# fzi-forschungszentrum-informatik/muvo

Hardware: AMD Instinct MI355X
Metric: world-model training samples/sec (seq_len=10) (higher is better)
Workload: dtype f32 storage/accumulate; large contractions (convolutions, transformer Linear) as bf16x3 split products

## Files before the change

### muvo_amd/csrc/conv_bf3.h

```cpp
#pragma once
#include "conv_plan.h"

void bf3_finish_phase(ConvPhase& g);
int bf3_pack_phase(const ConvPhase& g, const float* w, float* wp, hipStream_t st);
long bf3_workspace_bytes(int N, int C, long S);
int bf3_split_input(const float* x, void* ws, int N, int C, long S, hipStream_t st, const float* yact = nullptr, int act = 0,
                    float slope = 0.f, float* dbias = nullptr, const float* dhead = nullptr, const float* head_w = nullptr, int CO = 0,
                    float* dhead_w = nullptr, float* dhead_b = nullptr);
int bf3_launch_fwd_phase(const ConvPhase& g, const void* ws, const float* wp, const float* bias, float* out, int act,
                         float slope, hipStream_t st, int ksplit = 1);
void bf3_set_fused_head(const float* w, const float* b, float* out, int co);
void bf3_set_products(int n);
int bf3_get_products();
int bf3_fwd_ksplit(const ConvPhase& g);
int bf3_wgrad_phase(const ConvPhase& g, const void* ws_x, int Cin_total, const void* ws_dz, int Cout_total, float* wg,
                    float* dw, hipStream_t st);
int bf3_split_rows(const float* x, void* ws, long rows, int C, hipStream_t st);
bool bf3_fwd_uses_pp(const ConvPhase& g);
bool bf3_wgrad_uses_pp(const ConvPhase& g);
struct PackItem {
  ConvPhase g;
  const float* w;
  float* dst;
  long blk0;
  int nblk, pad_;
};
int pack_table_launch(const PackItem* dev_items, int n, long n_blocks, hipStream_t st);
```

### muvo_amd/csrc/conv_bf3.hip

```cpp
#include "conv_bf3.h"
#include <type_traits>

typedef __bf16 bf16x8 __attribute__((ext_vector_type(8)));
typedef __bf16 bf16x2 __attribute__((ext_vector_type(2)));
typedef float f32x2 __attribute__((ext_vector_type(2)));

__device__ unsigned long long g_bf3_clock[3];
extern "C" int muvo_bf3_loop_clock(double* shader_mhz, double* us_per_k_step) {
  unsigned long long h[3] = {0, 0, 0};
  if (hipMemcpyFromSymbol(h, HIP_SYMBOL(g_bf3_clock), sizeof(h)) != hipSuccess) return MUVO_ERR_HIP;
  if (h[1] == 0 || h[2] == 0) { *shader_mhz = 0.0; *us_per_k_step = 0.0; return MUVO_OK; }
  *shader_mhz = (double)h[0] / ((double)h[1] / 100.0);
  *us_per_k_step = (double)h[1] / 100.0 / (double)h[2];
  return MUVO_OK;
}

#ifdef MUVO_BF3_STAMPS
__device__ unsigned long long g_bf3_stamps[8 * 16384];
#define BF3_STAMP(slot)                                                                      \
  if (MUVO_BF3_STAMPS != 3 && threadIdx.x == 0 && blockIdx.x < 16384) g_bf3_stamps[blockIdx.x * 8 + (slot)] = __builtin_amdgcn_s_memrealtime()
extern "C" int muvo_debug_bf3_stamps_reset() {
  void* p = nullptr;
  return hipGetSymbolAddress(&p, HIP_SYMBOL(g_bf3_stamps)) == hipSuccess && hipMemset(p, 0, sizeof(unsigned long long) * 8 * 16384) == hipSuccess ? 0 : 1;
}
// ... 1250 lines not shown
    hipLaunchKernelGGL(nchw_split_nhwc_v4_kernel, grid, dim3(256), lds, st, x, hi, lo, C, Cp, S, yact, act, slope, dbias ? rep : nullptr,
                       dhead, head_w, CO, hw_rep, nrep);
  } else {
    hipLaunchKernelGGL(nchw_split_nhwc_kernel, grid, dim3(256), 0, st, x, hi, lo, C, Cp, S, yact, act, slope, rep, nrep);
  }
  if (dbias) hipLaunchKernelGGL(bias_replica_reduce_kernel, dim3(cdiv(Cp, 64)), dim3(64), 0, st, rep, dbias, C, Cp, nrep);
  if (hw_rep) hipLaunchKernelGGL(head_replica_reduce_kernel, dim3(cdiv(4 * Cp + 4, 64)), dim3(64), 0, st, hw_rep, dhead_w, dhead_b, C, Cp, CO, nrep);
  MUVO_CHECK_LAUNCH("nchw_split_nhwc_kernel");
  return MUVO_OK;
}

__global__ void __launch_bounds__(256) rows_split_kernel(const float* __restrict__ in, uint4* __restrict__ out_hi,
                                                         uint4* __restrict__ out_lo, long n_u4) {
  for (long i = blockIdx.x * 256L + threadIdx.x; i < n_u4; i += (long)gridDim.x * 256) {
    const float4 a = reinterpret_cast<const float4*>(in)[2 * i], b = reinterpret_cast<const float4*>(in)[2 * i + 1];
    uint4 h, l;
    split2(a.x, a.y, h.x, l.x);
    split2(a.z, a.w, h.y, l.y);
    split2(b.x, b.y, h.z, l.z);
    split2(b.z, b.w, h.w, l.w);
    out_hi[i] = h;
    out_lo[i] = l;
  }
  if (blockIdx.x == 0 && threadIdx.x == 0) out_hi[2 * n_u4] = make_uint4(0u, 0u, 0u, 0u);
}

int bf3_split_rows(const float* x, void* ws, long rows, int C, hipStream_t st) {
  const long n_u4 = rows * C / 8;
  uint4* hi = (uint4*)ws;
  hipLaunchKernelGGL(rows_split_kernel, dim3(ew_grid(n_u4)), dim3(256), 0, st, x, hi, hi + n_u4, n_u4);
  MUVO_CHECK_LAUNCH("rows_split_kernel");
  return MUVO_OK;
}

struct Bf3Head { const float* w; const float* b; float* out; int co; };
static thread_local Bf3Head t_bf3_head = {nullptr, nullptr, nullptr, 0};

static int g_bf3_products = 3;
void bf3_set_products(int n) { g_bf3_products = n == 1 ? 1 : 3; }
int bf3_get_products() { return g_bf3_products; }

template <int BM, int BN, int WM, int WN, int BKC, int NST, bool ONE>
static int bf3_launch_t(const ConvPhase& g, const void* ws, const float* wp, const float* bias, float* out, int act,
                        float slope, hipStream_t st, int ksplit) {
  constexpr size_t lds0 = (size_t)NST * 2 * BKC * (BM + BN) * 16 + 512 + 4 * BM * WN;
  static_assert(lds0 <= 160 * 1024, "LDS budget");
  constexpr size_t HEAD_LDS = NST == 3 ? 4096 : 0;
  const Bf3Head hd = (NST == 3 && ksplit <= 1) ? t_bf3_head : Bf3Head{nullptr, nullptr, nullptr, 0};
  const size_t lds = lds0 + (hd.co > 0 ? HEAD_LDS : 0);
  static_assert(lds0 + HEAD_LDS <= 160 * 1024, "LDS budget with a fused head");
  static bool attr_set = false;
  static const uint4* zero16 = nullptr;
  if (!attr_set) {
    if (hipFuncSetAttribute((const void*)conv_bf3_kernel<BM, BN, WM, WN, BKC, NST, ONE>, hipFuncAttributeMaxDynamicSharedMemorySize,
                            (int)(lds0 + HEAD_LDS)) != hipSuccess ||
        hipGetSymbolAddress((void**)&zero16, HIP_SYMBOL(g_zero16)) != hipSuccess) {
      muvo_set_error("conv_bf3: kernel attribute / symbol setup failed");
      return MUVO_ERR_HIP;
    }
    attr_set = true;
  }
  const long plane_u4 = (long)g.N * g.ID * g.IH * g.IW * (g.Cp / 8);
  dim3 grid(cdiv(g.npix, BN) * cdiv(g.M, BM), ksplit, 1);
  hipLaunchKernelGGL((conv_bf3_kernel<BM, BN, WM, WN, BKC, NST, ONE>), grid, dim3(64 * WM * WN), lds, st, g, (const uint4*)ws, plane_u4,
                     (const uint4*)wp, bias, out, act, slope, zero16, ksplit, hd.w, hd.b, hd.out, hd.co);
  MUVO_CHECK_LAUNCH("conv_bf3_kernel");
  return MUVO_OK;
}
template <int BM, int BN, int WM, int WN, int BKC, int NST>
static int bf3_launch(const ConvPhase& g, const void* ws, const float* wp, const float* bias, float* out, int act,
                      float slope, hipStream_t st, int ksplit = 1) {
  return g_bf3_products == 1 ? bf3_launch_t<BM, BN, WM, WN, BKC, NST, true>(g, ws, wp, bias, out, act, slope, st, ksplit)
                             : bf3_launch_t<BM, BN, WM, WN, BKC, NST, false>(g, ws, wp, bias, out, act, slope, st, ksplit);
}

bool bf3_fwd_uses_pp(const ConvPhase& g) {
  if (g.M <= 64) return false;
  const long big = g.M > 128 ? (long)cdiv(g.npix, 128) * cdiv(g.M, 256) : (long)cdiv(g.npix, 256) * cdiv(g.M, 128);
  static const int min_blocks = getenv("MUVO_BF3_PP_MIN_BLOCKS") ? atoi(getenv("MUVO_BF3_PP_MIN_BLOCKS")) : 128;
  return big >= min_blocks;
}
bool bf3_wgrad_uses_pp(const ConvPhase& g) { return g.M > 128 || (g.M > 64 && g.C > 64); }

int bf3_fwd_ksplit(const ConvPhase& g) {
  if (g.npix <= 0 || bf3_fwd_uses_pp(g) || muvo_det()) return 1;
  static const int tgt = getenv("MUVO_BF3_KSPLIT_BLOCKS") ? atoi(getenv("MUVO_BF3_KSPLIT_BLOCKS")) : 512;
  static const int min_steps = getenv("MUVO_BF3_KSPLIT_MIN_STEPS") ? atoi(getenv("MUVO_BF3_KSPLIT_MIN_STEPS")) : 16;
  const long tiles = (long)cdiv(g.npix, 128) * cdiv(g.M, 64);
  const int nk = g.Kp / 32;
  if (tiles >= 192 || nk < 2 * min_steps) return 1;
  int ks = cdiv(tgt, tiles);
  if (ks > nk / min_steps) ks = nk / min_steps;
  return ks < 1 ? 1 : ks;
}

void bf3_set_fused_head(const float* w, const float* b, float* out, int co) { t_bf3_head = Bf3Head{w, b, out, co}; }

int bf3_launch_fwd_phase(const ConvPhase& g, const void* ws, const float* wp, const float* bias, float* out, int act,
                         float slope, hipStream_t st, int ksplit) {
  if (g.npix <= 0) return MUVO_OK;
  if (ksplit > 1) return bf3_launch<64, 128, 1, 4, 4, 2>(g, ws, wp, nullptr, out, MUVO_ACT_NONE, 0.f, st, ksplit);
  static const int variant = getenv("MUVO_BF3_VARIANT") ? atoi(getenv("MUVO_BF3_VARIANT")) : 0;
  if (variant == 2) {
    if (g.M > 128) return bf3_launch<256, 128, 4, 2, 4, 2>(g, ws, wp, bias, out, act, slope, st);
    if (g.M > 64) return bf3_launch<128, 256, 2, 4, 4, 2>(g, ws, wp, bias, out, act, slope, st);
  }
  if (bf3_fwd_uses_pp(g)) {
    if (g.M > 128) return bf3_launch<256, 128, 4, 2, 4, 3>(g, ws, wp, bias, out, act, slope, st);
    return bf3_launch<128, 256, 2, 4, 4, 3>(g, ws, wp, bias, out, act, slope, st);
  }
  return bf3_launch<64, 128, 1, 4, 4, 2>(g, ws, wp, bias, out, act, slope, st);
}

static int bf3_wgrad_ksplit(long tiles, int nsteps, int tgt, int minst, int slots) {
  if (muvo_det()) return 1;
  int ksplit = cdiv(tgt, tiles);
  if (ksplit > cdiv(nsteps, minst)) ksplit = cdiv(nsteps, minst);
  if (ksplit < 1) ksplit = 1;
  static const int quant = getenv("MUVO_BF3_WGRAD_QUANT") ? atoi(getenv("MUVO_BF3_WGRAD_QUANT")) : 1;
  if (quant && tiles * ksplit < 4L * slots) {
    const int kmax = nsteps / 12 > 1 ? nsteps / 12 : 1;
    double best = 1e30;
    for (int ks = 1; ks <= kmax && tiles * ks <= 8L * slots; ++ks) {
      const int sps = cdiv(nsteps, ks);
      if (cdiv(nsteps, sps) != ks) continue;
      const double cost = (double)cdiv(tiles * ks, slots) * (sps * 1.2 + 12.0);
      if (cost < best - 1e-9) { best = cost; ksplit = ks; }
    }
  }
  return ksplit;
}

static int bf3_wgrad_xcd_order() {
  static const int v = getenv("MUVO_BF3_WGRAD_XCD") ? atoi(getenv("MUVO_BF3_WGRAD_XCD")) : 1;
  return v;
}

template <int BM, int BN, int WM, int WN, bool ONE>
static int bf3_wgrad_pp_launch_t(const ConvPhase& g, const void* ws_x, int Cin_total, const void* ws_dz, int Cout_total,
                                 float* wg, hipStream_t st) {
  constexpr size_t lds = (size_t)3 * 2 * 32 * (BM / 8 + BN / 8) * 16;
  static bool attr_set = false;
  if (!attr_set) {
    if (hipFuncSetAttribute((const void*)conv_bf3_wgrad_pp_kernel<BM, BN, WM, WN, ONE>, hipFuncAttributeMaxDynamicSharedMemorySize,
                            (int)lds) != hipSuccess) {
      muvo_set_error("conv_bf3_wgrad_pp: kernel attribute setup failed");
      return MUVO_ERR_HIP;
    }
    attr_set = true;
  }
  ConvPhase p = g;
  const int xc8 = roundup(Cin_total, 8) / 8, dzc8 = roundup(Cout_total, 8) / 8;
  p.Cp = xc8 * 8;
  const long xplane = (long)g.N * g.ID * g.IH * g.IW * xc8, dzplane = (long)g.N * g.OD * g.OH * g.OW * dzc8;
  const int ctiles = cdiv(g.C, BN), mtiles = cdiv(g.M, BM);
  const int nsteps = cdiv(g.npix, 32);
  static const int tgt = getenv("MUVO_BF3_WGRAD_PP_BLOCKS") ? atoi(getenv("MUVO_BF3_WGRAD_PP_BLOCKS")) : 2048;
  static const int minst = getenv("MUVO_BF3_WGRAD_PP_MINSTEPS") ? atoi(getenv("MUVO_BF3_WGRAD_PP_MINSTEPS")) : 32;
  int ksplit = bf3_wgrad_ksplit((long)ctiles * g.T * mtiles, nsteps, tgt, minst, 256);
  const int sps = cdiv(nsteps, ksplit);
  ksplit = cdiv(nsteps, sps);
  dim3 grid(ctiles * g.T, mtiles, ksplit);
  hipLaunchKernelGGL((conv_bf3_wgrad_pp_kernel<BM, BN, WM, WN, ONE>), grid, dim3(64 * WM * WN), lds, st, p, (const uint4*)ws_x, xplane,
                     xc8, (const uint4*)ws_dz, dzplane, dzc8, wg, sps, bf3_wgrad_xcd_order());
  MUVO_CHECK_LAUNCH("conv_bf3_wgrad_pp_kernel");
  return MUVO_OK;
}
template <int BM, int BN, int WM, int WN>
static int bf3_wgrad_pp_launch(const ConvPhase& g, const void* ws_x, int Cin_total, const void* ws_dz, int Cout_total,
                               float* wg, hipStream_t st) {
  return g_bf3_products == 1 ? bf3_wgrad_pp_launch_t<BM, BN, WM, WN, true>(g, ws_x, Cin_total, ws_dz, Cout_total, wg, st)
                             : bf3_wgrad_pp_launch_t<BM, BN, WM, WN, false>(g, ws_x, Cin_total, ws_dz, Cout_total, wg, st);
}

template <int BM, int BN, int WM, int WN, int WK, bool ONE>
static int bf3_wgrad_launch_t(const ConvPhase& g, const void* ws_x, int Cin_total, const void* ws_dz, int Cout_total,
                              float* wg, hipStream_t st) {
  constexpr size_t lds = (size_t)3 * 2 * 32 * (BM / 8 + BN / 8) * 16;
  static bool attr_set = false;
  static const uint4* zero16 = nullptr;
  if (!attr_set) {
    if (hipFuncSetAttribute((const void*)conv_bf3_wgrad_kernel<BM, BN, WM, WN, WK, ONE>, hipFuncAttributeMaxDynamicSharedMemorySize,
                            (int)lds) != hipSuccess ||
        hipGetSymbolAddress((void**)&zero16, HIP_SYMBOL(g_zero16)) != hipSuccess) {
// ... 65 lines not shown
```

### muvo_amd/csrc/conv_gemm.hip

```cpp
#include "common.h"
#include "conv_vox.h"
#include "conv_pw.h"
#include "conv_plan.h"
#include "conv_bf3.h"

typedef __bf16 wg_bf16x8 __attribute__((ext_vector_type(8)));
__device__ __forceinline__ void wg_split8(const float (&v)[8], wg_bf16x8& hi, wg_bf16x8& lo) {
  typedef __bf16 b2 __attribute__((ext_vector_type(2)));
  typedef float f2 __attribute__((ext_vector_type(2)));
  unsigned h[4], l[4];
#pragma unroll
  for (int p = 0; p < 4; ++p) {
    const b2 hh = __builtin_convertvector((f2){v[2 * p], v[2 * p + 1]}, b2);
    h[p] = __builtin_bit_cast(unsigned, hh);
    const float h0 = __uint_as_float(h[p] << 16), h1 = __uint_as_float(h[p] & 0xffff0000u);
    const b2 ll = __builtin_convertvector((f2){v[2 * p] - h0, v[2 * p + 1] - h1}, b2);
    l[p] = __builtin_bit_cast(unsigned, ll);
  }
  typedef unsigned u4 __attribute__((ext_vector_type(4)));
  hi = __builtin_bit_cast(wg_bf16x8, (u4){h[0], h[1], h[2], h[3]});
  lo = __builtin_bit_cast(wg_bf16x8, (u4){l[0], l[1], l[2], l[3]});
}

template <int BM, int BN, int WM, int WN, int RUN>
// ... 566 lines not shown
        int k = 0;
        while (k < nu && uni[k] != phs[i].tap_d[t]) ++k;
        if (k == nu) { if (nu < MAX_TAPS) uni[nu++] = phs[i].tap_d[t]; else fits = false; }
      }
    static const int min_pct = getenv("MUVO_MERGE_UNION_MIN_PCT") ? atoi(getenv("MUVO_MERGE_UNION_MIN_PCT")) : 50;
    const bool merge = same_grid && (same_taps || (allow_union && fits && nu > 1 && 100 * real >= min_pct * count * nu));
    if (merge) {
      ConvPhase g = phs[0];
      g.nmerge = count;
      g.Msub = M;
      g.M = count * M;
      g.T = nu;
      for (int t = 0; t < nu; ++t) g.tap_d[t] = uni[t];
      for (int i = 0; i < count; ++i) {
        for (int a = 0; a < 3; ++a) g.mop[i][a] = phs[i].op[a];
        for (int t = 0; t < nu; ++t) {
          int k = 0;
          while (k < phs[i].T && phs[i].tap_d[k] != uni[t]) ++k;
          g.tap_wm[i][t] = k < phs[i].T ? phs[i].tap_w[k] : -1;
        }
      }
      for (int t = 0; t < nu; ++t) g.tap_w[t] = g.tap_wm[0][t] >= 0 ? g.tap_wm[0][t] : 0;
      finish_phase(g);
      phs[0] = g;
      count = 1;
    }
  }
  *nph = count;
  return MUVO_OK;
}

struct ConvPlan {
  ConvPhase fwd[8]; int nfwd;
  ConvPhase dgr[8]; int ndgr;
  long fwd_floats, dgr_floats;
};

static int build_plan(const muvo_conv_desc* d, ConvPlan* pl, int mode = -1, bool allow_merge = true) {
  int rc = check_desc(d);
  if (rc) return rc;
  t_plan_mode = mode < 0 ? conv_mode() : mode;
  t_allow_merge = allow_merge;
  const long taps = (long)d->ksz[0] * d->ksz[1] * d->ksz[2];
  if (!d->transposed) {
    pl->nfwd = 1;
    rc = build_conv_form(d, d->in_sz, d->out_sz, d->Cin, d->Cout, d->Cin * taps, taps, &pl->fwd[0]);
    if (rc) return rc;
    rc = build_transposed_form(d, d->out_sz, d->in_sz, d->Cout, d->Cin, taps, d->Cin * taps, pl->dgr, &pl->ndgr);
    if (rc) return rc;
  } else {
    rc = build_transposed_form(d, d->in_sz, d->out_sz, d->Cin, d->Cout, taps, d->Cout * taps, pl->fwd, &pl->nfwd);
    if (rc) return rc;
    pl->ndgr = 1;
    rc = build_conv_form(d, d->out_sz, d->in_sz, d->Cout, d->Cin, d->Cout * taps, taps, &pl->dgr[0]);
    if (rc) return rc;
  }
  long off = 0;
  for (int i = 0; i < pl->nfwd; ++i) { pl->fwd[i].wp_off = off; off += (long)pl->fwd[i].Kp * pl->fwd[i].Mp; }
  pl->fwd_floats = off;
  off = 0;
  for (int i = 0; i < pl->ndgr; ++i) { pl->dgr[i].wp_off = off; off += (long)pl->dgr[i].Kp * pl->dgr[i].Mp; }
  pl->dgr_floats = off;
  return MUVO_OK;
}

static double f32_bf3_min_gflop() {
  static const double v = getenv("MUVO_F32_BF3_MIN_GFLOP") ? atof(getenv("MUVO_F32_BF3_MIN_GFLOP")) : 2.0;
  return v;
}

template <int BM, int BN, int WM, int WN>
static void launch_fwd_run(const ConvPhase& g, const float* in, const float* wp, const float* bias, float* out,
                           int act, float slope, hipStream_t st, int ksplit) {
  dim3 grid(cdiv(g.npix, BN), cdiv(g.M, BM), ksplit);
  constexpr int KPT = 16 / (256 / BN);
  if (g.Cp == 4)
    hipLaunchKernelGGL((conv_fwd_kernel<BM, BN, WM, WN, 4>), grid, dim3(256), 0, st, g, in, wp, bias, out, act, slope, ksplit);
  else if (g.Cp == 8 || KPT == 8)
    hipLaunchKernelGGL((conv_fwd_kernel<BM, BN, WM, WN, 8>), grid, dim3(256), 0, st, g, in, wp, bias, out, act, slope, ksplit);
  else
    hipLaunchKernelGGL((conv_fwd_kernel<BM, BN, WM, WN, KPT>), grid, dim3(256), 0, st, g, in, wp, bias, out, act, slope, ksplit);
}

static int phase_ksplit(const ConvPhase& g) {
  if (g.npix <= 0 || muvo_det()) return 1;
  if (g.bf3) return bf3_fwd_ksplit(g);
  const int bm = g.M > 64 ? 128 : (g.M > 32 ? 64 : 32);
  const long blocks = (long)cdiv(g.npix, 128) * cdiv(g.M, bm);
  const int nk = g.Kp / 16;
  static const int min_steps = getenv("MUVO_KSPLIT_MIN_STEPS") ? atoi(getenv("MUVO_KSPLIT_MIN_STEPS")) : 8;
  if (blocks >= 192 || nk < 4 * min_steps) return 1;
  static const int ks_tgt = getenv("MUVO_KSPLIT_BLOCKS") ? atoi(getenv("MUVO_KSPLIT_BLOCKS")) : 384;
  int ks = cdiv(ks_tgt, blocks);
  if (ks > nk / min_steps) ks = nk / min_steps;
  return ks < 1 ? 1 : ks;
}

static int launch_fwd_phase(const ConvPhase& g, const float* in, const float* wp, const float* bias, float* out,
                            int act, float slope, hipStream_t st, const void* ws, int ksplit) {
  if (g.npix <= 0) return MUVO_OK;
  if (g.bf3) return bf3_launch_fwd_phase(g, ws, wp, bias, out, act, slope, st, ksplit);
  if (g.M > 64) launch_fwd_run<128, 128, 2, 2>(g, in, wp, bias, out, act, slope, st, ksplit);
  else if (g.M > 32) launch_fwd_run<64, 128, 2, 2>(g, in, wp, bias, out, act, slope, st, ksplit);
  else launch_fwd_run<32, 128, 1, 4>(g, in, wp, bias, out, act, slope, st, ksplit);
  MUVO_CHECK_LAUNCH("conv_fwd_kernel");
  return MUVO_OK;
}

static int launch_wgrad_phase(const ConvPhase& g, const float* in, const float* dout, float* dwp, hipStream_t st) {
  if (g.npix <= 0 || g.T == 0) return MUVO_OK;
  const int ntiles = cdiv(g.npix, 32);
  const int rows = g.Kp;
  int bm, bn;
  if (g.M > 64) bn = 128; else if (g.M > 32) bn = 64; else bn = 32;
  bm = 128;
  const int gx = cdiv(rows, bm), gy = cdiv(g.M, bn);
  static const int tgt = getenv("MUVO_F32_WGRAD_BLOCKS") ? atoi(getenv("MUVO_F32_WGRAD_BLOCKS")) : 2048;
  static const int mint = getenv("MUVO_F32_WGRAD_MINTILES") ? atoi(getenv("MUVO_F32_WGRAD_MINTILES")) : 4;
  int nsplit = cdiv(tgt, gx * gy);
  if (nsplit > cdiv(ntiles, mint)) nsplit = cdiv(ntiles, mint);
  if (nsplit < 1 || muvo_det()) nsplit = 1;
  const int tps = cdiv(ntiles, nsplit);
  nsplit = cdiv(ntiles, tps);
  dim3 grid(gx, gy, nsplit);
  static const bool want_bf3 = !getenv("MUVO_F32_WGRAD_BF3") || atoi(getenv("MUVO_F32_WGRAD_BF3")) != 0;
  const bool b3 = want_bf3 && conv_mode() == 1 &&
                  2e-9 * (double)g.M * (double)g.npix * (double)g.T * (double)g.C >= f32_bf3_min_gflop();
  if (b3) {
    if (bn == 128) hipLaunchKernelGGL((conv_wgrad_kernel<128, 128, 2, 2, true>), grid, dim3(256), 0, st, g, in, dout, dwp, tps);
    else if (bn == 64) hipLaunchKernelGGL((conv_wgrad_kernel<128, 64, 2, 2, true>), grid, dim3(256), 0, st, g, in, dout, dwp, tps);
    else hipLaunchKernelGGL((conv_wgrad_kernel<128, 32, 4, 1, true>), grid, dim3(256), 0, st, g, in, dout, dwp, tps);
  } else {
    if (bn == 128) hipLaunchKernelGGL((conv_wgrad_kernel<128, 128, 2, 2, false>), grid, dim3(256), 0, st, g, in, dout, dwp, tps);
    else if (bn == 64) hipLaunchKernelGGL((conv_wgrad_kernel<128, 64, 2, 2, false>), grid, dim3(256), 0, st, g, in, dout, dwp, tps);
    else hipLaunchKernelGGL((conv_wgrad_kernel<128, 32, 4, 1, false>), grid, dim3(256), 0, st, g, in, dout, dwp, tps);
  }
  MUVO_CHECK_LAUNCH("conv_wgrad_kernel");
  return MUVO_OK;
}

extern "C" {

int muvo_conv_set_mode(int mode) {
  MUVO_CHECK_ARG(mode == MUVO_CONV_F32 || mode == MUVO_CONV_BF16X3, "conv_set_mode: unknown mode %d", mode);
  g_conv_mode = mode;
  return MUVO_OK;
}
int muvo_conv_get_mode(void) { return conv_mode(); }
int muvo_conv_set_products(int n) {
  MUVO_CHECK_ARG(n == 1 || n == 3, "conv_set_products: 1 (bf16) or 3 (bf16x3), got %d", n);
  bf3_set_products(n);
  return MUVO_OK;
}
int muvo_conv_get_products(void) { return bf3_get_products(); }
int muvo_conv_set_bf16x3_min_gflop(double gflop_per_item) {
  g_bf3_min_gflop = gflop_per_item < 0.0 ? -1.0 : gflop_per_item;
  return MUVO_OK;
}

int muvo_conv_pack_sizes(const muvo_conv_desc* d, int64_t* fwd_floats, int64_t* dgrad_floats) {
  ConvPlan pl;
  int rc = build_plan(d, &pl);
  if (rc) return rc;
  {
    ConvPlan pf;
    rc = build_plan(d, &pf, 0, false);
    if (rc) return rc;
    if (pf.fwd_floats > pl.fwd_floats) pl.fwd_floats = pf.fwd_floats;
  }
// ... 30 lines not shown
    wp_dgrad = nullptr;
  }
  if (wp_fwd)
    for (int i = 0; i < pl.nfwd; ++i) {
      const long total = (long)pl.fwd[i].Kp * pl.fwd[i].Mp;
      if (total == 0) continue;
      if (pl.fwd[i].bf3) {
        rc = bf3_pack_phase(pl.fwd[i], w, wp_fwd, st);
        if (rc) return rc;
        continue;
      }
      hipLaunchKernelGGL(pack_weights_kernel, dim3(ew_grid(total)), dim3(256), 0, st, pl.fwd[i], w, wp_fwd);
    }
  if (wp_dgrad)
    for (int i = 0; i < pl.ndgr; ++i) {
      const long total = (long)pl.dgr[i].Kp * pl.dgr[i].Mp;
      if (total == 0) continue;
      if (pl.dgr[i].bf3) {
        rc = bf3_pack_phase(pl.dgr[i], w, wp_dgrad, st);
        if (rc) return rc;
        continue;
      }
      hipLaunchKernelGGL(pack_weights_kernel, dim3(ew_grid(total)), dim3(256), 0, st, pl.dgr[i], w, wp_dgrad);
    }
  MUVO_CHECK_LAUNCH("pack_weights_kernel");
  return MUVO_OK;
}

static bool wgrad_uses_bf3(const ConvPlan& pf);
int64_t muvo_conv_workspace_bytes(const muvo_conv_desc* d, int op) {
  ConvPlan pl;
  if (op >= 2) {
    if (build_plan(d, &pl, 0, false)) return -1;
    if (pw_applicable(d) || vox_wgrad_ok(d) || !wgrad_uses_bf3(pl)) return 0;
    return op == 2 ? bf3_workspace_bytes(d->N, d->Cin, (long)d->in_sz[0] * d->in_sz[1] * d->in_sz[2])
                   : bf3_workspace_bytes(d->N, d->Cout, (long)d->out_sz[0] * d->out_sz[1] * d->out_sz[2]);
  }
  if (build_plan(d, &pl)) return -1;
  const ConvPhase* ph = op == 0 ? pl.fwd : pl.dgr;
  const int nph = op == 0 ? pl.nfwd : pl.ndgr;
  if (pw_applicable(d)) return 0;
  if (op == 0 ? vox_fwd_ok(d) : vox_dgrad_ok(d)) return 0;
  for (int i = 0; i < nph; ++i)
    if (ph[i].bf3) return bf3_workspace_bytes(ph[i].N, ph[i].C, (long)ph[i].ID * ph[i].IH * ph[i].IW);
  return 0;
}

int muvo_conv_kernel_family(const muvo_conv_desc* d, int op) {
  ConvPlan pl;
  if (pw_applicable(d)) return 3;
  if (op == 2) {
    if (build_plan(d, &pl, 0, false)) return -1;
    if (vox_wgrad_ok(d)) return vox_wgrad_uses_bf3(d) ? 4 : 2;
    return wgrad_uses_bf3(pl) ? 1 : 0;
  }
  if (build_plan(d, &pl)) return -1;
  if (op == 0 ? vox_fwd_ok(d) : vox_dgrad_ok(d)) return vox_uses_bf3(d, op) ? 4 : 2;
  const ConvPhase* ph = op == 0 ? pl.fwd : pl.dgr;
  const int nph = op == 0 ? pl.nfwd : pl.ndgr;
  for (int i = 0; i < nph; ++i)
    if (ph[i].bf3) return 1;
  return 0;
}

int muvo_conv_kernel_variant(const muvo_conv_desc* d, int op) {
  if (muvo_conv_kernel_family(d, op) != 1) return 0;
  ConvPlan pl;
  if (op == 2) {
    if (build_plan(d, &pl, 0, true) || !wgrad_uses_bf3(pl)) {
      if (build_plan(d, &pl, 0, false)) return 0;
    }
    return pl.nfwd > 0 && bf3_wgrad_uses_pp(pl.fwd[0]) ? 1 : 0;
  }
  if (build_plan(d, &pl)) return 0;
  const ConvPhase* ph = op == 0 ? pl.fwd : pl.dgr;
  const int nph = op == 0 ? pl.nfwd : pl.ndgr;
  return nph > 0 && bf3_fwd_uses_pp(ph[0]) ? 1 : 0;
}

static int run_phases(const ConvPhase* ph, int nph, const float* in, const float* wp, const float* bias, float* out, int act,
                      float slope, void* ws, hipStream_t st, bool ws_valid = false) {
  bool split_done = ws_valid;
  static const int any_rule = getenv("MUVO_KSPLIT_ANY") ? atoi(getenv("MUVO_KSPLIT_ANY")) : 1;
  bool use_ksplit = nph > 0 && !any_rule, any_ks = false;
  for (int i = 0; i < nph; ++i) {
    use_ksplit = use_ksplit && phase_ksplit(ph[i]) > 1;
    any_ks = any_ks || phase_ksplit(ph[i]) > 1;
  }
  if (any_rule) use_ksplit = any_ks;
  const long out_total = nph > 0 ? (long)ph[0].N * ph[0].out_sN : 0;
  if (use_ksplit && hipMemsetAsync(out, 0, sizeof(float) * out_total, st) != hipSuccess) {
    muvo_set_error("conv: memset of the split-K output failed");
    return MUVO_ERR_HIP;
  }
  for (int i = 0; i < nph; ++i) {
    if (ph[i].bf3 && !split_done) {
      MUVO_CHECK_ARG(ws != nullptr, "conv: this shape runs on the bf16x3 kernel and needs muvo_conv_workspace_bytes() of workspace");
      int rc = bf3_split_input(in, ws, ph[i].N, ph[i].C, (long)ph[i].ID * ph[i].IH * ph[i].IW, st);
      if (rc) return rc;
      split_done = true;
    }
    const int ks_i = phase_ksplit(ph[i]);
    int rc = launch_fwd_phase(ph[i], in, wp, bias, out, act, slope, st, ws, use_ksplit ? (ks_i > 1 ? ks_i : 2) : 1);
    if (rc) return rc;
  }
  if (use_ksplit && (bias != nullptr || act != MUVO_ACT_NONE)) {
    hipLaunchKernelGGL(bias_act_kernel, dim3(ew_grid(out_total)), dim3(256), 0, st, out, bias, ph[0].Msub, (long)ph[0].out_sC,
                       out_total, act, slope);
    MUVO_CHECK_LAUNCH("bias_act_kernel");
  }
  return MUVO_OK;
}

int muvo_conv_forward(const muvo_conv_desc* d, const float* x, const float* wp_fwd, const float* bias, float* y,
                      int act, float slope, void* ws, void* stream) {
  ConvPlan pl;
  int rc = build_plan(d, &pl);
  if (rc) return rc;
  MUVO_CHECK_ARG(x && wp_fwd && y, "conv_forward: null pointer");
  if (pw_applicable(d)) return pw_forward(d, x, wp_fwd, bias, y, act, slope, (hipStream_t)stream);
  if (vox_fwd_ok(d)) return vox_forward(d, x, wp_fwd, bias, y, act, slope, (hipStream_t)stream, vox_uses_bf3(d, 0));
  return run_phases(pl.fwd, pl.nfwd, x, wp_fwd, bias, y, act, slope, ws, (hipStream_t)stream);
}

int muvo_conv_forward_planes(const muvo_conv_desc* d, const float* x, const float* wp_fwd, const float* bias, float* y, int act,
                             float slope, void* ws, int ws_valid, void* stream) {
  if (!ws_valid) return muvo_conv_forward(d, x, wp_fwd, bias, y, act, slope, ws, stream);
  ConvPlan pl;
  int rc = build_plan(d, &pl);
  if (rc) return rc;
  MUVO_CHECK_ARG(wp_fwd && y && ws, "conv_forward_planes: null pointer");
  MUVO_CHECK_ARG(!pw_applicable(d) && !vox_fwd_ok(d), "conv_forward_planes: this shape does not read split planes");
  bool all_bf3 = pl.nfwd > 0;
  for (int i = 0; i < pl.nfwd; ++i) all_bf3 = all_bf3 && pl.fwd[i].bf3;
  MUVO_CHECK_ARG(all_bf3, "conv_forward_planes: ws_valid needs every phase on the bf16x3 kernels (muvo_conv_kernel_family == 1)");
  return run_phases(pl.fwd, pl.nfwd, x, wp_fwd, bias, y, act, slope, ws, (hipStream_t)stream, true);
}

int muvo_conv_forward_head_supported(const muvo_conv_desc* d, int CO) {
  if (check_desc(d) || CO < 1 || CO > 4) return 0;
  static const int on = getenv("MUVO_CONV_HEAD_FWD") ? atoi(getenv("MUVO_CONV_HEAD_FWD")) : 1;
  if (!on || muvo_det() || conv_mode() != 1 || pw_applicable(d) || vox_fwd_ok(d)) return 0;
  ConvPlan pl;
  if (build_plan(d, &pl) != MUVO_OK || pl.nfwd < 1) return 0;
  for (int i = 0; i < pl.nfwd; ++i) {
    const ConvPhase& g = pl.fwd[i];
    if (!g.bf3 || !bf3_fwd_uses_pp(g) || phase_ksplit(g) > 1) return 0;
    if (g.Msub != d->Cout || g.Msub % 64 != 0 || g.M % 64 != 0 || (long)CO * g.Msub > 1024) return 0;
    if ((long)g.N * g.out_sN * 4 >= 0x7fffff00L) return 0;
  }
  return 1;
}
int muvo_conv_forward_head(const muvo_conv_desc* d, const float* x, const float* wp_fwd, const float* bias, float* y, int act,
                           float slope, void* ws, const float* head_w, const float* head_b, int CO, float* logits, void* stream) {
  ConvPlan pl;
  int rc = build_plan(d, &pl);
  if (rc) return rc;
  MUVO_CHECK_ARG(x && wp_fwd && y && head_w && logits, "conv_forward_head: null pointer");
  MUVO_CHECK_ARG(muvo_conv_forward_head_supported(d, CO), "conv_forward_head: shape not served by the eight-wave bf16x3 tiles");
  hipStream_t st = (hipStream_t)stream;
  if (d->Cout > 64) {
    const long S_out = (long)d->out_sz[0] * d->out_sz[1] * d->out_sz[2];
    if (hipMemsetAsync(logits, 0, sizeof(float) * (size_t)d->N * CO * S_out, st) != hipSuccess) {
      muvo_set_error("conv_forward_head: memset of the logits failed");
      return MUVO_ERR_HIP;
    }
  }
  bf3_set_fused_head(head_w, head_b, logits, CO);
  rc = run_phases(pl.fwd, pl.nfwd, x, wp_fwd, bias, y, act, slope, ws, st);
  bf3_set_fused_head(nullptr, nullptr, nullptr, 0);
  return rc;
}

int muvo_conv_forward_moments_supported(const muvo_conv_desc* d) {
  if (check_desc(d)) return 0;
  if (muvo_det()) return 0;
  return (!pw_applicable(d) && vox_fwd_ok(d) && vox_uses_bf3(d, 0)) ? 1 : 0;
}
int muvo_conv_forward_moments(const muvo_conv_desc* d, const float* x, const float* wp_fwd, const float* bias, float* y, int act,
                              float slope, double* moments, void* stream) {
  ConvPlan pl;
  int rc = build_plan(d, &pl);
  if (rc) return rc;
  MUVO_CHECK_ARG(x && wp_fwd && y && moments, "conv_forward_moments: null pointer");
  MUVO_CHECK_ARG(muvo_conv_forward_moments_supported(d), "conv_forward_moments: only the bf16x3 voxel kernels produce output moments");
  return vox_forward(d, x, wp_fwd, bias, y, act, slope, (hipStream_t)stream, true, moments);
}

int muvo_conv_affine_supported(const muvo_conv_desc* d) {
  if (check_desc(d)) return 0;
  return (conv_mode() == 1 && !pw_applicable(d) && vox_fwd_ok(d) && vox_uses_bf3(d, 0) && vox_wgrad_applicable(d) &&
          vox_wgrad_uses_bf3(d) && vox_affine_ok(d)) ? 1 : 0;
}
int muvo_conv_forward_affine(const muvo_conv_desc* d, const float* x, const float* aff, const float* wp_fwd, const float* bias,
                             float* y, int act, float slope, double* moments, void* stream) {
  ConvPlan pl;
  int rc = build_plan(d, &pl);
  if (rc) return rc;
  MUVO_CHECK_ARG(x && aff && wp_fwd && y, "conv_forward_affine: null pointer");
  MUVO_CHECK_ARG(muvo_conv_affine_supported(d), "conv_forward_affine: shape not served by the bf16x3 voxel kernels");
  return vox_forward(d, x, wp_fwd, bias, y, act, slope, (hipStream_t)stream, true, moments, aff);
}
int muvo_conv_wgrad_affine(const muvo_conv_desc* d, const float* x, const float* aff, const float* dy, float* dw, float* dbias,
                           void* stream) {
  ConvPlan pl;
  int rc = build_plan(d, &pl, 0, false);
  if (rc) return rc;
  MUVO_CHECK_ARG(x && aff && dy && dw, "conv_wgrad_affine: null pointer");
  MUVO_CHECK_ARG(muvo_conv_affine_supported(d), "conv_wgrad_affine: shape not served by the bf16x3 voxel kernels");
  return vox_wgrad(d, x, dy, dw, dbias, (hipStream_t)stream, true, aff);
}

int muvo_conv_dgrad(const muvo_conv_desc* d, const float* dy, const float* wp_dgrad, float* dx, void* ws, int ws_valid,
                    void* stream) {
  ConvPlan pl;
  int rc = build_plan(d, &pl);
  if (rc) return rc;
  MUVO_CHECK_ARG(dy && wp_dgrad && dx, "conv_dgrad: null pointer");
  if (pw_applicable(d)) return pw_dgrad(d, dy, wp_dgrad, dx, (hipStream_t)stream);
  if (vox_dgrad_ok(d)) return vox_dgrad(d, dy, wp_dgrad, dx, (hipStream_t)stream, vox_uses_bf3(d, 1));
  return run_phases(pl.dgr, pl.ndgr, dy, wp_dgrad, nullptr, dx, MUVO_ACT_NONE, 0.f, ws, (hipStream_t)stream, ws_valid != 0);
}

int muvo_conv_dgrad_accumulate(const muvo_conv_desc* d, const float* dy, const float* wp_dgrad, float* dx, void* stream) {
  int rc = check_desc(d);
  if (rc) return rc;
  MUVO_CHECK_ARG(dy && wp_dgrad && dx, "conv_dgrad_accumulate: null pointer");
  MUVO_CHECK_ARG(pw_applicable(d), "conv_dgrad_accumulate: only the 1x1 head kernels (muvo_conv_kernel_family == 3) accumulate");
  return pw_dgrad_acc(d, dy, wp_dgrad, dx, (hipStream_t)stream);
}
// ... 267 lines not shown
```

Baseline: 26.27.

## Choose bf16x3 forward K-split with a cost model, extending split to pingpong tiles

Replaces the fixed K-split heuristic for bf16x3 forward convolutions with an analytic cost model. The model estimates per-step and fixed costs against occupancy slots, adds the cost of reduction traffic and an optional bias/activation finish pass, and picks the cheapest split. Pingpong (eight-wave) tiles, which were never split before, can now be split, and split launches keep their large tile shapes. Per-phase split factors are computed once and cached, and the fused-head path now opts out of splitting. The risk is the extra atomic/reduction traffic and finish pass when the model's hand-fitted constants mispredict.

```diff
diff --git a/muvo_amd/csrc/conv_bf3.h b/muvo_amd/csrc/conv_bf3.h
--- a/muvo_amd/csrc/conv_bf3.h
+++ b/muvo_amd/csrc/conv_bf3.h
@@ -12,7 +12,7 @@
 void bf3_set_fused_head(const float* w, const float* b, float* out, int co);
 void bf3_set_products(int n);
 int bf3_get_products();
-int bf3_fwd_ksplit(const ConvPhase& g);
+int bf3_fwd_ksplit(const ConvPhase& g, bool finish_pass);
 int bf3_wgrad_phase(const ConvPhase& g, const void* ws_x, int Cin_total, const void* ws_dz, int Cout_total, float* wg,
                     float* dw, hipStream_t st);
 int bf3_split_rows(const float* x, void* ws, long rows, int C, hipStream_t st);
diff --git a/muvo_amd/csrc/conv_bf3.hip b/muvo_amd/csrc/conv_bf3.hip
--- a/muvo_amd/csrc/conv_bf3.hip
+++ b/muvo_amd/csrc/conv_bf3.hip
@@ -1356,24 +1356,86 @@
 }
 bool bf3_wgrad_uses_pp(const ConvPhase& g) { return g.M > 128 || (g.M > 64 && g.C > 64); }
 
-int bf3_fwd_ksplit(const ConvPhase& g) {
-  if (g.npix <= 0 || bf3_fwd_uses_pp(g) || muvo_det()) return 1;
+static int bf3_fwd_split_mode() {
+  const char* e = getenv("MUVO_BF3_FWD_SPLIT");
+  return e ? atoi(e) : 1;
+}
+
+static int bf3_fwd_ksplit_v0(long tiles, int nk, int min_steps) {
   static const int tgt = getenv("MUVO_BF3_KSPLIT_BLOCKS") ? atoi(getenv("MUVO_BF3_KSPLIT_BLOCKS")) : 512;
-  static const int min_steps = getenv("MUVO_BF3_KSPLIT_MIN_STEPS") ? atoi(getenv("MUVO_BF3_KSPLIT_MIN_STEPS")) : 16;
-  const long tiles = (long)cdiv(g.npix, 128) * cdiv(g.M, 64);
-  const int nk = g.Kp / 32;
-  if (tiles >= 192 || nk < 2 * min_steps) return 1;
+  if (tiles >= 192) return 1;
   int ks = cdiv(tgt, tiles);
   if (ks > nk / min_steps) ks = nk / min_steps;
   return ks < 1 ? 1 : ks;
 }
 
+static double lerp3(const double (&v)[3], double r) {
+  if (r <= 1.0) return v[0];
+  if (r >= 3.0) return v[2];
+  const int i = (int)r - 1;
+  return v[i] + (v[i + 1] - v[i]) * (r - (i + 1));
+}
+
+int bf3_fwd_ksplit(const ConvPhase& g, bool finish_pass) {
+  if (g.npix <= 0 || muvo_det() || t_bf3_head.co > 0) return 1;
+  static const int min_steps = getenv("MUVO_BF3_KSPLIT_MIN_STEPS") ? atoi(getenv("MUVO_BF3_KSPLIT_MIN_STEPS")) : 16;
+  const int nk = g.Kp / 32;
+  if (nk < 2 * min_steps) return 1;
+  const bool pp = bf3_fwd_uses_pp(g);
+  const long tiles = !pp ? (long)cdiv(g.npix, 128) * cdiv(g.M, 64)
+                         : (g.M > 128 ? (long)cdiv(g.npix, 128) * cdiv(g.M, 256) : (long)cdiv(g.npix, 256) * cdiv(g.M, 128));
+  const long slots = pp ? 256 : 768;
+  if (tiles >= (pp ? 2 * slots : slots)) return 1;
+  const int mode = bf3_fwd_split_mode();
+  if (mode == 0) return pp ? 1 : bf3_fwd_ksplit_v0(tiles, nk, min_steps);
+  const int kmax = nk / min_steps;
+  if (mode >= 2) return mode < kmax ? mode : kmax;
+  if (!pp) {
+    if (tiles < 192) return bf3_fwd_ksplit_v0(tiles, nk, min_steps);
+  } else {
+    static const int pp_on = getenv("MUVO_BF3_FWD_SPLIT_PP") ? atoi(getenv("MUVO_BF3_FWD_SPLIT_PP")) : 1;
+    if (!pp_on) return 1;
+  }
+  for (int a = 0; a < 3; ++a)
+    if (g.os[a] != 1 || (!pp && g.is[a] != 1)) return 1;
+  static const double step_small[3] = {0.80, 0.93, 1.18}, fixed_small[3] = {8.4, 14.9, 30.9};
+  const double out_mb = (double)g.N * g.out_sN * 4.0 * 1e-6;
+  double best = 1e30, unsplit = 1e30;
+  int best_ks = 1;
+  for (int ks = 1; ks <= kmax && tiles * ks <= 4 * slots; ++ks) {
+    const int sps = cdiv(nk, ks);
+    if (cdiv(nk, sps) != ks) continue;
+    const long wgs = tiles * ks;
+    const double busy = (double)(wgs < slots ? wgs : slots) / 256.0;
+    double t_step, t_fixed;
+    if (pp) {
+      const double f = busy <= 0.5 ? 0.0 : (busy - 0.5) * 2.0;
+      t_step = 0.93 + f * (1.20 - 0.93);
+      t_fixed = 10.5 + f * (13.6 - 10.5);
+    } else {
+      t_step = lerp3(step_small, busy);
+      t_fixed = lerp3(fixed_small, busy);
+    }
+    double cost = (double)cdiv(wgs, slots) * (sps * t_step + t_fixed);
+    if (ks == 1) unsplit = cost;
+    else cost += 3.0 + out_mb / 3.0 + 0.5 * ks * out_mb / 1.3 + (finish_pass ? 3.0 + 2.0 * out_mb / 3.0 : 0.0);
+    if (cost < best - 1e-9) { best = cost; best_ks = ks; }
+  }
+  return best < 0.95 * unsplit ? best_ks : 1;
+}
+
 void bf3_set_fused_head(const float* w, const float* b, float* out, int co) { t_bf3_head = Bf3Head{w, b, out, co}; }
 
 int bf3_launch_fwd_phase(const ConvPhase& g, const void* ws, const float* wp, const float* bias, float* out, int act,
                          float slope, hipStream_t st, int ksplit) {
   if (g.npix <= 0) return MUVO_OK;
-  if (ksplit > 1) return bf3_launch<64, 128, 1, 4, 4, 2>(g, ws, wp, nullptr, out, MUVO_ACT_NONE, 0.f, st, ksplit);
+  if (ksplit > 1) {
+    if (bf3_fwd_uses_pp(g) && bf3_fwd_split_mode() != 0) {
+      if (g.M > 128) return bf3_launch<256, 128, 4, 2, 4, 3>(g, ws, wp, nullptr, out, MUVO_ACT_NONE, 0.f, st, ksplit);
+      return bf3_launch<128, 256, 2, 4, 4, 3>(g, ws, wp, nullptr, out, MUVO_ACT_NONE, 0.f, st, ksplit);
+    }
+    return bf3_launch<64, 128, 1, 4, 4, 2>(g, ws, wp, nullptr, out, MUVO_ACT_NONE, 0.f, st, ksplit);
+  }
   static const int variant = getenv("MUVO_BF3_VARIANT") ? atoi(getenv("MUVO_BF3_VARIANT")) : 0;
   if (variant == 2) {
     if (g.M > 128) return bf3_launch<256, 128, 4, 2, 4, 2>(g, ws, wp, bias, out, act, slope, st);
diff --git a/muvo_amd/csrc/conv_gemm.hip b/muvo_amd/csrc/conv_gemm.hip
--- a/muvo_amd/csrc/conv_gemm.hip
+++ b/muvo_amd/csrc/conv_gemm.hip
@@ -672,9 +672,9 @@
     hipLaunchKernelGGL((conv_fwd_kernel<BM, BN, WM, WN, KPT>), grid, dim3(256), 0, st, g, in, wp, bias, out, act, slope, ksplit);
 }
 
-static int phase_ksplit(const ConvPhase& g) {
+static int phase_ksplit(const ConvPhase& g, bool finish_pass) {
   if (g.npix <= 0 || muvo_det()) return 1;
-  if (g.bf3) return bf3_fwd_ksplit(g);
+  if (g.bf3) return bf3_fwd_ksplit(g, finish_pass);
   const int bm = g.M > 64 ? 128 : (g.M > 32 ? 64 : 32);
   const long blocks = (long)cdiv(g.npix, 128) * cdiv(g.M, bm);
   const int nk = g.Kp / 16;
@@ -871,10 +871,14 @@
                       float slope, void* ws, hipStream_t st, bool ws_valid = false) {
   bool split_done = ws_valid;
   static const int any_rule = getenv("MUVO_KSPLIT_ANY") ? atoi(getenv("MUVO_KSPLIT_ANY")) : 1;
+  const bool finish_pass = bias != nullptr || act != MUVO_ACT_NONE;
+  int ks[8];
+  MUVO_CHECK_ARG(nph <= 8, "conv: too many phases");
   bool use_ksplit = nph > 0 && !any_rule, any_ks = false;
   for (int i = 0; i < nph; ++i) {
-    use_ksplit = use_ksplit && phase_ksplit(ph[i]) > 1;
-    any_ks = any_ks || phase_ksplit(ph[i]) > 1;
+    ks[i] = phase_ksplit(ph[i], finish_pass);
+    use_ksplit = use_ksplit && ks[i] > 1;
+    any_ks = any_ks || ks[i] > 1;
   }
   if (any_rule) use_ksplit = any_ks;
   const long out_total = nph > 0 ? (long)ph[0].N * ph[0].out_sN : 0;
@@ -889,11 +893,10 @@
       if (rc) return rc;
       split_done = true;
     }
-    const int ks_i = phase_ksplit(ph[i]);
-    int rc = launch_fwd_phase(ph[i], in, wp, bias, out, act, slope, st, ws, use_ksplit ? (ks_i > 1 ? ks_i : 2) : 1);
-    if (rc) return rc;
-  }
-  if (use_ksplit && (bias != nullptr || act != MUVO_ACT_NONE)) {
+    int rc = launch_fwd_phase(ph[i], in, wp, bias, out, act, slope, st, ws, use_ksplit ? (ks[i] > 1 ? ks[i] : 2) : 1);
+    if (rc) return rc;
+  }
+  if (use_ksplit && finish_pass) {
     hipLaunchKernelGGL(bias_act_kernel, dim3(ew_grid(out_total)), dim3(256), 0, st, out, bias, ph[0].Msub, (long)ph[0].out_sC,
                        out_total, act, slope);
     MUVO_CHECK_LAUNCH("bias_act_kernel");
@@ -934,7 +937,7 @@
   if (build_plan(d, &pl) != MUVO_OK || pl.nfwd < 1) return 0;
   for (int i = 0; i < pl.nfwd; ++i) {
     const ConvPhase& g = pl.fwd[i];
-    if (!g.bf3 || !bf3_fwd_uses_pp(g) || phase_ksplit(g) > 1) return 0;
+    if (!g.bf3 || !bf3_fwd_uses_pp(g)) return 0;
     if (g.Msub != d->Cout || g.Msub % 64 != 0 || g.M % 64 != 0 || (long)CO * g.Msub > 1024) return 0;
     if ((long)g.N * g.out_sN * 4 >= 0x7fffff00L) return 0;
   }
```

After: 26.35 (median of 6 runs). Within noise of the previous version (+0.3%).
